# vliu15/3d-brain-tumor-segmentation

Hardware: AMD Instinct MI355X
Metric: training volumes/sec (2ch x 128^3) (higher is better)
Workload: dtype f32; 1 GPU; BASELINE configs[1]: 2ch x 128^3, batch 1 per GPU, fp32, full fwd+bwd with Dice+KL+L2 VAE loss + Dice metric + TF-form Adam; CLI-default model (base_filters=32, depth=4, groups=8, reduction=8; 42,174,773 params); parallelism=dp1, global_batch=1

## Files before the change

### 3d-brain-tumor-segmentation_amd/csrc/conv_wgrad.hip

```cpp
#include <stdlib.h>
#include <type_traits>
#include "common.h"
#include "bts_internal.h"

int bts_prof_on();
void bts_prof_begin(int sym, double flops, hipStream_t stream);
void bts_prof_end(hipStream_t stream);

#define WG_THREADS 512
#define WG_WAVES 8
#define WG_MAXT 4
#define WG_PSLOTS 8
#define WG_QSLOTS 4

struct WgradParams {
  const float* p;
  const float* q;
  float* partial;
  double* partial_b;
  const float* zeros;
  int N, Dp, Hp, Wp, Cp, ldp;
  int Dq, Hq, Wq, Cq, ldq;
  int s, loz, loy, lox;
  int IZ, IY, IX;
// ... 736 lines not shown
      if (c < bestc - 1e-9) { bestc = c; best = n; }
    }
    if (best > p.nsub) best = p.nsub;
    p.sub_per_wg = (int)((p.nsub + best - 1) / best);
    pl.nsp = (p.nsub + p.sub_per_wg - 1) / p.sub_per_wg;
  }
  pl.partial_floats = (long)pl.nsp * pl.npct * pl.nqct * p.ntiles * 1024;
  pl.partial_b_doubles = (long)pl.nsp * pl.nqct * 32;
  return BTS_OK;
}

typedef float wg_f32x2 __attribute__((ext_vector_type(2)));
__device__ __forceinline__ wg_f32x2 wgw_pk_add(wg_f32x2 a, wg_f32x2 b) { wg_f32x2 d; asm("v_pk_add_f32 %0, %1, %2" : "=v"(d) : "v"(a), "v"(b)); return d; }
__device__ __forceinline__ wg_f32x2 wgw_pk_sub(wg_f32x2 a, wg_f32x2 b) { wg_f32x2 d; asm("v_pk_add_f32 %0, %1, %2 neg_lo:[0,1] neg_hi:[0,1]" : "=v"(d) : "v"(a), "v"(b)); return d; }
__device__ __forceinline__ wg_f32x2 wgw_pk_fma(wg_f32x2 a, wg_f32x2 b, wg_f32x2 c) { wg_f32x2 d; asm("v_pk_fma_f32 %0, %1, %2, %3" : "=v"(d) : "v"(a), "v"(b), "v"(c)); return d; }
__device__ __forceinline__ f32x4 wgw_add4(f32x4 a, f32x4 b) { const wg_f32x2 lo = wgw_pk_add(a.xy, b.xy), hi = wgw_pk_add(a.zw, b.zw); return f32x4{lo.x, lo.y, hi.x, hi.y}; }
__device__ __forceinline__ f32x4 wgw_sub4(f32x4 a, f32x4 b) { const wg_f32x2 lo = wgw_pk_sub(a.xy, b.xy), hi = wgw_pk_sub(a.zw, b.zw); return f32x4{lo.x, lo.y, hi.x, hi.y}; }
__device__ __forceinline__ f32x4 wgw_fma4(f32x4 a, wg_f32x2 s, f32x4 c) { const wg_f32x2 lo = wgw_pk_fma(a.xy, s, c.xy), hi = wgw_pk_fma(a.zw, s, c.zw); return f32x4{lo.x, lo.y, hi.x, hi.y}; }
__device__ __forceinline__ float wgw_acc_rd(float a) { float v; asm volatile("v_accvgpr_read_b32 %0, %1" : "=v"(v) : "a"(a)); return v; }

#define WGW_QSTR 28
#define WGW_PTILE (24 * 32 * 16)
#define WGW_QTILE (8 * 32 * WGW_QSTR)
#define WGW_BUF (WGW_PTILE + WGW_QTILE)
#define WGW_NPS 12
#define WGW_NQS 5
#define WGW_THREADS 256

__global__ __launch_bounds__(WGW_THREADS, 1) void wgw_kernel(const WgradParams p) {
  extern __shared__ __attribute__((aligned(16))) float lds[];
  const int tid = threadIdx.x;
  const int lane = tid & 63;
  const int wave = __builtin_amdgcn_readfirstlane(tid >> 6);
  const int ch = lane & 31, hh = lane >> 5;
  const int pct = blockIdx.y, qct = blockIdx.z;
  const float* pP = p.p + pct * 32;
  const float* pQ = p.q + qct * 32;

  const int sxx = tid & 15, scq = (tid >> 4) & 7, srow0 = tid >> 7;
  const int p_lds0 = (srow0 * 32 + scq * 4) * 16 + ((((sxx >> 2) ^ (scq & 3)) << 2) | (sxx & 3));
  unsigned poff[WGW_NPS], pfl0 = 0, pfl1 = 0;
#pragma unroll
  for (int i = 0; i < WGW_NPS; ++i) {
    const int row = srow0 + 2 * i;
    const int zr = row / 6, yr = row - zr * 6;
    poff[i] = (unsigned)(((zr * p.Hp + yr) * p.Wp + sxx) * p.ldp + scq * 4) * 4u;
    const unsigned fl = (zr == 0 ? 1u : 0u) | (zr == 3 ? 2u : 0u) | (yr == 0 ? 4u : 0u) | (yr == 5 ? 8u : 0u);
    if (i < 8) pfl0 |= fl << (4 * i); else pfl1 |= fl << (4 * (i - 8));
  }
  int q_lds[WGW_NQS];
  unsigned qoff[WGW_NQS], qfl = 0;
#pragma unroll
  for (int i = 0; i < WGW_NQS; ++i) {
    const int id = tid + WGW_THREADS * i;
    q_lds[i] = -1; qoff[i] = 0x80000000u;
    if (id < 1152) {
      const int xx = id % 18, kq = (id / 18) & 7, row = id / 144;
      q_lds[i] = WGW_PTILE + (row * 32 + kq * 4) * WGW_QSTR + xx + 3;
      qoff[i] = (unsigned)((((row >> 2) * p.Hq + (row & 3)) * p.Wq + xx) * p.ldq + kq * 4) * 4u;
      qfl |= ((xx == 0 ? 1u : 0u) | (xx == 17 ? 2u : 0u)) << (2 * i);
    }
  }
  int ftx, fty, ftz, fn;
  {
    int t = blockIdx.x * p.sub_per_wg;
    ftx = t % p.ntx; t /= p.ntx;
    fty = t % p.nty; t /= p.nty;
    ftz = t % p.ntz;
    fn = t / p.ntz;
  }
  f32x4 pre[WGW_NPS + WGW_NQS];
  __amdgpu_buffer_rsrc_t f_pr, f_qr;
  unsigned f_tm = 0, f_qm = 0;
  auto fetch_begin = [&]() {
    const int z0 = 2 * ftz, y0 = 4 * fty, x0 = 16 * ftx;
    const float* pb = pP + ((((long)fn * p.Dp + z0 - 1) * p.Hp + y0 - 1) * p.Wp + x0) * p.ldp;
    const float* qb = pQ + ((((long)fn * p.Dq + z0) * p.Hq + y0) * p.Wq + x0 - 1) * p.ldq;
    f_pr = __builtin_amdgcn_make_buffer_rsrc((void*)pb, 0, 0x7fffffff, 0x00020000);
    f_qr = __builtin_amdgcn_make_buffer_rsrc((void*)qb, 0, 0x7fffffff, 0x00020000);
    f_tm = (ftz == 0 ? 1u : 0u) | (ftz == p.ntz - 1 ? 2u : 0u) | (fty == 0 ? 4u : 0u) | (fty == p.nty - 1 ? 8u : 0u);
    f_qm = (ftx == 0 ? 1u : 0u) | (ftx == p.ntx - 1 ? 2u : 0u);
    if (++ftx == p.ntx) { ftx = 0; if (++fty == p.nty) { fty = 0; if (++ftz == p.ntz) { ftz = 0; ++fn; } } }
  };
  auto fetch_p = [&](auto ic) {
    constexpr int i = decltype(ic)::value;
    constexpr int sh = 4 * (i & 7);
    const unsigned fl = (((i < 8 ? pfl0 : pfl1) >> sh) & 15u) & f_tm;
    pre[i] = __builtin_bit_cast(f32x4, __builtin_amdgcn_raw_buffer_load_b128(f_pr, fl ? 0x80000000u : poff[i], 0, 0));
  };
  auto fetch_q = [&](auto ic) {
    constexpr int i = decltype(ic)::value;
    const unsigned fl = ((qfl >> (2 * i)) & 3u) & f_qm;
    pre[WGW_NPS + i] = __builtin_bit_cast(f32x4, __builtin_amdgcn_raw_buffer_load_b128(f_qr, fl ? 0x80000000u : qoff[i], 0, 0));
  };
  auto commit_p = [&](float* buf, auto ic) {
    constexpr int i = decltype(ic)::value;
#pragma unroll
    for (int e = 0; e < 4; ++e) buf[p_lds0 + i * (2 * 32 * 16) + e * 16] = pre[i][e];
  };
  auto commit_q = [&](float* buf, auto ic) {
    constexpr int i = decltype(ic)::value;
    if (q_lds[i] >= 0) {
#pragma unroll
      for (int e = 0; e < 4; ++e) buf[q_lds[i] + e * WGW_QSTR] = pre[WGW_NPS + i][e];
    }
  };
  auto fetch_quarter = [&](auto kc) {
    constexpr int k = decltype(kc)::value;
    fetch_p(IC<3 * k>{}); fetch_p(IC<3 * k + 1>{}); fetch_p(IC<3 * k + 2>{});
    if constexpr (k == 0) { fetch_q(IC<0>{}); fetch_q(IC<1>{}); } else fetch_q(IC<k + 1>{});
  };
  auto commit_quarter = [&](float* buf, auto kc) {
    constexpr int k = decltype(kc)::value;
    commit_p(buf, IC<3 * k>{}); commit_p(buf, IC<3 * k + 1>{}); commit_p(buf, IC<3 * k + 2>{});
    if constexpr (k == 0) { commit_q(buf, IC<0>{}); commit_q(buf, IC<1>{}); } else commit_q(buf, IC<k + 1>{});
  };

  const int ra = (wave == 0) ? 0 : (wave == 2) ? 2 : 1;
  const int rb = (wave == 0) ? 2 : (wave == 1) ? 2 : (wave == 2) ? 1 : 3;
  const float sp = (wave == 1) ? 1.f : -1.f;
  const wg_f32x2 sp2 = {sp, sp};
  const float sq = (wave == 1) ? 1.f : (wave == 2) ? -1.f : 0.f;
  const wg_f32x2 sq2 = {sq, sq};
  const int qX = (wave == 3) ? 4 * 32 * WGW_QSTR : 0;
  const int pswz = (ch >> 2) & 3;
  const int pA = (ra * 6 * 32 + ch) * 16, pB = (rb * 6 * 32 + ch) * 16;
  const bool bias = p.want_bias && pct == 0 && wave == 1;
  double bsum = 0.0;

  f32x16 acc[3][4];
#pragma unroll
  for (int a = 0; a < 3; ++a)
#pragma unroll
    for (int c = 0; c < 4; ++c)
#pragma unroll
      for (int r = 0; r < 16; ++r) acc[a][c][r] = 0.f;

  struct WgwOps {
    f32x4 v[4];
    f32x4 a0, a1, u1, u2;
    float a0s[2], a1s[2], u1s[2], u2s[2];
  };
  auto form = [&](const float* cur, auto stc, WgwOps& o) {
    constexpr int st = decltype(stc)::value;
    constexpr int py2 = st >> 1, sx = st & 1;
    const int xq = 2 * sx + hh;
    const int xo = 4 * xq;
    const int pq = (xq ^ pswz) << 2;
    f32x4 c[4];
#pragma unroll
    for (int yr = 0; yr < 4; ++yr) {
      const f32x4 a = *reinterpret_cast<const f32x4*>(cur + pA + (2 * py2 + yr) * 512 + pq);
      const f32x4 b = *reinterpret_cast<const f32x4*>(cur + pB + (2 * py2 + yr) * 512 + pq);
      c[yr] = wgw_fma4(b, sp2, a);
    }
    o.v[0] = wgw_sub4(c[0], c[2]);
    o.v[1] = wgw_add4(c[1], c[2]);
    o.v[2] = wgw_sub4(c[2], c[1]);
    o.v[3] = wgw_sub4(c[1], c[3]);
    const float* qb = cur + WGW_PTILE + ((2 * py2) * 32 + ch) * WGW_QSTR + xo;
    {
      const f32x4 x0q = *reinterpret_cast<const f32x4*>(qb + qX + 4);
      const f32x4 x1q = *reinterpret_cast<const f32x4*>(qb + qX + 32 * WGW_QSTR + 4);
      const f32x4 y0q = *reinterpret_cast<const f32x4*>(qb + (4 * 32) * WGW_QSTR + 4);
      const f32x4 y1q = *reinterpret_cast<const f32x4*>(qb + (5 * 32) * WGW_QSTR + 4);
      o.a0 = wgw_fma4(y0q, sq2, x0q);
      o.a1 = wgw_fma4(y1q, sq2, x1q);
      o.u1 = wgw_add4(o.a0, o.a1);
      o.u2 = wgw_sub4(o.a0, o.a1);
      if (bias) bsum += (double)((o.u1[0] + o.u1[1]) + (o.u1[2] + o.u1[3]));
    }
#pragma unroll
    for (int e = 0; e < 2; ++e) {
      const int off = e == 0 ? 0 : 8, el = e == 0 ? 3 : 0;
      f32x4 xs0 = *reinterpret_cast<const f32x4*>(qb + qX + off);
      f32x4 xs1 = *reinterpret_cast<const f32x4*>(qb + qX + 32 * WGW_QSTR + off);
      f32x4 ys0 = *reinterpret_cast<const f32x4*>(qb + (4 * 32) * WGW_QSTR + off);
      f32x4 ys1 = *reinterpret_cast<const f32x4*>(qb + (5 * 32) * WGW_QSTR + off);
      asm volatile("" : "+v"(xs0), "+v"(xs1), "+v"(ys0), "+v"(ys1));
      o.a0s[e] = fmaf(ys0[el], sq, xs0[el]);
      o.a1s[e] = fmaf(ys1[el], sq, xs1[el]);
      o.u1s[e] = o.a0s[e] + o.a1s[e];
      o.u2s[e] = o.a0s[e] - o.a1s[e];
    }
  };
  auto mfma48 = [&](const WgwOps& o) {
#pragma unroll
    for (int dx = 0; dx < 3; ++dx)
#pragma unroll
      for (int j = 0; j < 4; ++j) {
        const int w = 5 + j - dx;
        const float b0 = w == 3 ? o.a0s[0] : w == 8 ? o.a0s[1] : o.a0[(w - 4) & 3];
        const float b1 = w == 3 ? o.u1s[0] : w == 8 ? o.u1s[1] : o.u1[(w - 4) & 3];
        const float b2 = w == 3 ? o.u2s[0] : w == 8 ? o.u2s[1] : o.u2[(w - 4) & 3];
        const float b3 = w == 3 ? o.a1s[0] : w == 8 ? o.a1s[1] : o.a1[(w - 4) & 3];
        acc[dx][0] = __builtin_amdgcn_mfma_f32_32x32x2f32(o.v[0][j], b0, acc[dx][0], 0, 0, 0);
        acc[dx][1] = __builtin_amdgcn_mfma_f32_32x32x2f32(o.v[1][j], b1, acc[dx][1], 0, 0, 0);
        acc[dx][2] = __builtin_amdgcn_mfma_f32_32x32x2f32(o.v[2][j], b2, acc[dx][2], 0, 0, 0);
        acc[dx][3] = __builtin_amdgcn_mfma_f32_32x32x2f32(o.v[3][j], b3, acc[dx][3], 0, 0, 0);
      }
  };
#define WGW_SCHED_STEP()                                   \
  _Pragma("unroll") for (int q_ = 0; q_ < 48; ++q_) {      \
    __builtin_amdgcn_sched_group_barrier(0x008, 1, 0);     \
    __builtin_amdgcn_sched_group_barrier(0x002, 2, 0);     \
    __builtin_amdgcn_sched_group_barrier(0x320, 1, 0);     \
  }

  const int t0 = blockIdx.x * p.sub_per_wg;
  int t1 = t0 + p.sub_per_wg;
  if (t1 > p.nsub) t1 = p.nsub;
  if (t0 < t1) {
    fetch_begin();
    fetch_quarter(IC<0>{}); fetch_quarter(IC<1>{}); fetch_quarter(IC<2>{}); fetch_quarter(IC<3>{});
    commit_quarter(lds, IC<0>{}); commit_quarter(lds, IC<1>{}); commit_quarter(lds, IC<2>{}); commit_quarter(lds, IC<3>{});
  }
  __syncthreads();
  WgwOps opA, opB;
  for (int t = t0; t < t1; ++t) {
    const float* cur = lds + ((t - t0) & 1) * WGW_BUF;
    float* nxt = lds + ((t - t0 + 1) & 1) * WGW_BUF;
    const bool more = (t + 1) < t1;
    form(cur, IC<0>{}, opA);
    if (more) fetch_begin();
    __builtin_amdgcn_sched_barrier(0);
    asm volatile("s_nop 3" ::: "memory");
    if (more) fetch_quarter(IC<0>{});
    form(cur, IC<1>{}, opB);
    mfma48(opA);
    WGW_SCHED_STEP();
    __builtin_amdgcn_sched_barrier(0);
    asm volatile("s_nop 1" ::: "memory");
    if (more) { commit_quarter(nxt, IC<0>{}); fetch_quarter(IC<1>{}); }
    form(cur, IC<2>{}, opA);
    mfma48(opB);
    WGW_SCHED_STEP();
    __builtin_amdgcn_sched_barrier(0);
    asm volatile("s_nop 1" ::: "memory");
    if (more) { commit_quarter(nxt, IC<1>{}); fetch_quarter(IC<2>{}); }
    form(cur, IC<3>{}, opB);
    mfma48(opA);
    WGW_SCHED_STEP();
    __builtin_amdgcn_sched_barrier(0);
    asm volatile("s_nop 1" ::: "memory");
    if (more) { commit_quarter(nxt, IC<2>{}); fetch_quarter(IC<3>{}); }
    mfma48(opB);
    WGW_SCHED_STEP();
    __builtin_amdgcn_sched_barrier(0);
    if (more) commit_quarter(nxt, IC<3>{});
    __syncthreads();
  }

  asm volatile("s_nop 15\n\ts_nop 15\n\ts_nop 15\n\ts_nop 15\n\ts_nop 15" ::: "memory");
  float* xl = lds + wave * 9 * 1024;
#pragma unroll
  for (int dx = 0; dx < 3; ++dx)
#pragma unroll
    for (int r = 0; r < 16; ++r) {
      const float u0 = wgw_acc_rd(acc[dx][0][r]), u1 = wgw_acc_rd(acc[dx][1][r]), u2 = wgw_acc_rd(acc[dx][2][r]),
                  u3 = wgw_acc_rd(acc[dx][3][r]);
      const float hs = 0.5f * (u1 + u2), hd = 0.5f * (u1 - u2);
      const int crow = 8 * (r >> 2) + 4 * hh + (r & 3);
      float* o = xl + (dx * 3) * 1024 + crow * 32 + ch;
      o[0] = u0 + hs;
      o[1024] = hd;
      o[2048] = hs - u3;
    }
  __syncthreads();
  float* out = p.partial + ((((long)blockIdx.x * gridDim.y + pct) * gridDim.z + qct) * 27) * 1024;
  for (int e = tid; e < 9 * 1024; e += WGW_THREADS) {
    const int g = e >> 10, ck = e & 1023;
    const int dx = g / 3, ky = g - dx * 3;
    const float l0 = lds[(0 * 9 + g) * 1024 + ck], l1 = lds[(1 * 9 + g) * 1024 + ck], l2 = lds[(2 * 9 + g) * 1024 + ck],
                l3 = lds[(3 * 9 + g) * 1024 + ck];
    const float hs = 0.5f * (l1 + l2), hd = 0.5f * (l1 - l2);
    out[((0 * 3 + ky) * 3 + dx) * 1024 + ck] = l0 + hs;
    out[((1 * 3 + ky) * 3 + dx) * 1024 + ck] = hd;
    out[((2 * 3 + ky) * 3 + dx) * 1024 + ck] = hs - l3;
  }
  if (bias) {
    const double o = __shfl_xor(bsum, 32, 64);
    if (lane < 32) p.partial_b[((long)blockIdx.x * gridDim.z + qct) * 32 + ch] = bsum + o;
  }
}

#define K1W_THREADS 512
#define K1W_U 8
__global__ __launch_bounds__(K1W_THREADS, 2) void k1w_kernel(const WgradParams p, long NV, long chunk) {
  __shared__ float lds[8 * 1024];
  const int tid = threadIdx.x;
  const int lane = tid & 63;
  const int wave = __builtin_amdgcn_readfirstlane(tid >> 6);
  const int ch = lane & 31, hh = lane >> 5;
// ... 63 lines not shown
  r.ntaps = (kind == BTS_CONV_K1) ? 1 : 27;
  r.s = 1; r.neg = 0; r.swapped = 0; r.transposed = 0;
  r.Dp = D; r.Hp = H; r.Wp = W; r.Cp = Cin; r.Dq = D; r.Hq = H; r.Wq = W; r.Cq = Cout;
  if (kind == BTS_CONV_K3S2) {
    if ((D | H | W) & 1) return BTS_ERR_SHAPE;
    r.s = 2; r.Dq = D / 2; r.Hq = H / 2; r.Wq = W / 2;
  } else if (kind == BTS_CONV_K3S2T) {
    r.transposed = 1;
    r.s = 2; r.Dp = 2 * D; r.Hp = 2 * H; r.Wp = 2 * W; r.Cp = Cout; r.Cq = Cin;
  } else if (kind == BTS_CONV_K3S1 && Cout <= 8 && Cin > Cout) {
    r.swapped = 1; r.neg = 1; r.Cp = Cout; r.Cq = Cin;
  }
  return BTS_OK;
}

extern "C" int bts_colsum(const float* x, float* out, void* workspace, long workspace_bytes, int N, long rows, int C,
                          int ld, float scale, int sum_over_n, int accumulate, hipStream_t stream);
extern "C" long bts_colsum_workspace(int N, long rows, int C);

extern "C" long bts_conv3d_bwd_weight_workspace(int kind, int N, int D, int H, int W, int Cin, int Cout) {
  WgradRoles r;
  if (wgrad_roles(r, kind, D, H, W, Cin, Cout) != BTS_OK) return -1;
  WgradPlan pl;
  if (plan_wgrad(pl, r.ntaps, r.s, r.neg, N, r.Dp, r.Hp, r.Wp, r.Cp, r.Dq, r.Hq, r.Wq, r.Cq) != BTS_OK) return -1;
  const long base = ((pl.partial_floats * 4 + pl.partial_b_doubles * 8 + 256 + 15) & ~15L);
  return base + (r.swapped ? bts_colsum_workspace(N, (long)D * H * W, Cout) : 0) + 128;
}

extern "C" int bts_conv3d_bwd_weight(int kind, const float* x, const float* dy, float* dw, float* db, void* workspace,
                                     long workspace_bytes, int N, int D, int H, int W, int Cin, int ldx, int Cout,
                                     int lddy, int dup_start, int dup_shift, int accumulate, hipStream_t stream) {
  WgradRoles ro;
  int r = wgrad_roles(ro, kind, D, H, W, Cin, Cout);
  if (r != BTS_OK) return r;
  if (dup_shift > 0 && (kind == BTS_CONV_K3S2 || kind == BTS_CONV_K3S2T)) return BTS_ERR_UNSUPPORTED;
  WgradPlan pl;
  r = plan_wgrad(pl, ro.ntaps, ro.s, ro.neg, N, ro.Dp, ro.Hp, ro.Wp, ro.Cp, ro.Dq, ro.Hq, ro.Wq, ro.Cq);
  if (r != BTS_OK) return r;
  const long need = bts_conv3d_bwd_weight_workspace(kind, N, D, H, W, Cin, Cout);
  if (workspace_bytes < need || workspace == nullptr) return BTS_ERR_WORKSPACE;
  WgradParams& p = pl.p;
// ... 9 lines not shown
  p.want_bias = (db != nullptr && !pIsDy) ? 1 : 0;
  typedef void (*WgKernel)(const WgradParams);
  static const WgKernel kernels[4] = {wgrad_kernel<0, 0>, wgrad_kernel<1, 0>, wgrad_kernel<2, 1>, wgrad_kernel<2, 2>};
  static bool attr_done = false;
  if (!attr_done) {
    for (int i = 0; i < 4; ++i) {
      hipError_t e = hipFuncSetAttribute(reinterpret_cast<const void*>(kernels[i]), hipFuncAttributeMaxDynamicSharedMemorySize, 160 * 1024);
      if (e != hipSuccess) return (int)e;
    }
    attr_done = true;
  }
  char* ztail = reinterpret_cast<char*>(workspace) + ((need - 64) & ~15L);
  p.zeros = reinterpret_cast<const float*>(ztail);
  const bool glds = (p.ldp % 4 == 0) && (p.Cp % 4 == 0) && ((((uintptr_t)p.p) & 15) == 0) && (p.ldq % 4 == 0) &&
                    (p.Cq % 4 == 0) && ((((uintptr_t)p.q) & 15) == 0);
  if (p.fastf && ((double)p.IZ * p.Hp * p.Wp * p.ldp * 4.0 >= 4.0e9 || (double)p.TZ * p.Hq * p.Wq * p.ldq * 4.0 >= 4.0e9 || !glds))
    p.fastf = p.fixg = 0;
  const bool prof = bts_prof_on();
  if (glds && !p.fastf) {
    hipError_t e = hipMemsetAsync(ztail, 0, 64, stream);
    if (e != hipSuccess) return (int)e;
  }
  const int kidx = !glds ? 0 : (p.fastf ? 1 + p.fixg : 1);
  bool use_wgw = false;
  if (kidx == 2 && ro.ntaps == 27 && ro.s == 1) {
    const char* e = getenv("BTS_WGW");
    use_wgw = !(e && atoi(e) == 0) && 5.0 * p.Hp * p.Wp * p.ldp * 4.0 < 2.0e9 && 3.0 * p.Hq * p.Wq * p.ldq * 4.0 < 2.0e9;
  }
  bool use_k1w = false;
  const long NVall = (long)N * ro.Dq * ro.Hq * ro.Wq;
  if (ro.ntaps == 1 && !pIsDy && p.ntiles == 1 && NVall >= 32768) {
    const char* e = getenv("BTS_K1W");
    use_k1w = !(e && atoi(e) == 0);
  }
  if (use_k1w) {
    const long chunk = (((NVall + pl.nsp - 1) / pl.nsp) + 15) & ~15L;
    if (prof) bts_prof_begin(26, 2.0 * (double)ro.Cp * ro.Cq * (double)NVall, stream);
    (void)hipGetLastError();
    hipLaunchKernelGGL(k1w_kernel, dim3(pl.nsp, pl.npct, pl.nqct), dim3(K1W_THREADS), 0, stream, p, NVall, chunk);
    if (prof) bts_prof_end(stream);
    BTS_LAUNCH_CHECK();
  } else if (use_wgw) {
    static bool wattr = false;
    if (!wattr) {
      hipError_t e = hipFuncSetAttribute(reinterpret_cast<const void*>(wgw_kernel), hipFuncAttributeMaxDynamicSharedMemorySize, 160 * 1024);
      if (e != hipSuccess) return (int)e;
      wattr = true;
    }
    if (prof) bts_prof_begin(24, 2.0 * ro.ntaps * (double)ro.Cp * ro.Cq * (double)N * ro.Dq * ro.Hq * ro.Wq, stream);
    (void)hipGetLastError();
    hipLaunchKernelGGL(wgw_kernel, dim3(pl.nsp, pl.npct, pl.nqct), dim3(WGW_THREADS), (size_t)2 * WGW_BUF * sizeof(float), stream, p);
    if (prof) bts_prof_end(stream);
    BTS_LAUNCH_CHECK();
  } else {
  static const int ksym[4] = {100, 104, 109, 110};
  if (prof) bts_prof_begin(ksym[kidx], 2.0 * ro.ntaps * (double)ro.Cp * ro.Cq * (double)N * ro.Dq * ro.Hq * ro.Wq, stream);
  (void)hipGetLastError(); hipLaunchKernelGGL(kernels[kidx], dim3(pl.nsp, pl.npct, pl.nqct), dim3(WG_THREADS), pl.shmem, stream, p);
// ... 33 lines not shown
```

### 3d-brain-tumor-segmentation_amd/ops.py

```python
import ctypes
import weakref

import numpy as np
import torch

from ._lib import ERRORS, lib

K1, K3S1, K3S2, K3S2T = 0, 1, 2, 3
ROLE_FWD, ROLE_BWD = 0, 1
FLAG_SIGMOID, FLAG_ACCUM = 1, 2
GN_SLAB, GN_CHANNEL = 0, 1

_workspaces = {}

_CFG = {0: '2,1,4,1', 1: '2,2,4,1', 2: '1,2,2,2', 3: '1,1,2,2', 4: '1,1,4,1'}


_VARIANTS = {33: {1: '<0,5>', 2: '<0,4>', 3: '<1,5>', 4: '<1,4>'},
             32: {1: '<3x3x3>', 2: '<1x1x1>'}}


def kernel_symbol(sym, detail=False):
    var, sym = sym >> 16, sym & 0xffff
    if var and detail and sym in _VARIANTS:
# ... 312 lines not shown
        lib().call('bts_conv3d_bwd_data', kind, _p(dy), _p(wp_bwd), _p(dx), _p(ws), nb, n, d, h, w, cin, ld_of(dx), cout,
                   ld_of(dy), FLAG_ACCUM if accumulate else 0, _stream())
    return dx


def conv_bwd_weight(kind, x, dy, dw, db, dup_start=0, dup_shift=0, accumulate=False):
    n, d, h, w, cin = x.shape
    cout = dy.shape[4]
    nb = lib().query('bts_conv3d_bwd_weight_workspace', kind, n, d, h, w, cin, cout)
    ws = workspace(nb, x.device)
    if True:
        lib().call('bts_conv3d_bwd_weight', kind, _p(x), _p(dy), _p(dw), _p(db), _p(ws), nb, n, d, h, w, cin, ld_of(x),
                   cout, ld_of(dy), dup_start, dup_shift, 1 if accumulate else 0, _stream())


def gn_stats(x, groups, mode, eps=1e-5):
    if not x.is_contiguous():
        raise RuntimeError('GroupNormalization statistics need a dense tensor')
    n, c = x.shape[0], x.shape[4]
    v = x.shape[1] * x.shape[2] * x.shape[3]
    nb = lib().query('bts_gn_workspace', n, v, c, groups, mode)
    ws = workspace(nb, x.device)
    mean = torch.empty(n * groups, dtype=torch.float32, device=x.device)
    rstd = torch.empty_like(mean)
    lib().call('bts_gn_stats', _p(x), _p(mean), _p(rstd), _p(ws), nb, n, v, c, groups, mode, eps, _stream())
    return mean, rstd


def gn_apply(x, gamma, beta, mean, rstd, groups, mode, relu, out=None):
    n, c = x.shape[0], x.shape[4]
# ... 1001 lines not shown
```

### include/bts_hip.h

```cpp
#ifndef BTS_HIP_H
#define BTS_HIP_H
#include <stdint.h>
#ifdef __cplusplus
extern "C" {
#endif

typedef struct ihipStream_t* bts_stream_t;

#define BTS_OK 0
#define BTS_ERR_SHAPE (-1)
#define BTS_ERR_ALIGN (-2)
#define BTS_ERR_UNSUPPORTED (-3)
#define BTS_ERR_WORKSPACE (-4)
#define BTS_ERR_RCCL_BASE (-100)

#define BTS_CONV_K1 0
#define BTS_CONV_K3S1 1
#define BTS_CONV_K3S2 2
#define BTS_CONV_K3S2T 3
#define BTS_ROLE_FWD 0
#define BTS_ROLE_BWD_DATA 1
#define BTS_CONV_FLAG_SIGMOID 1
#define BTS_CONV_FLAG_ACCUM 2

// ... 17 lines not shown
int bts_conv3d_fwd_can_fuse(int N, int D, int H, int W, int Cin, int Cout);
int bts_conv3d_fwd_fused2(const float* x, const float* wp_fwd, const float* bias, float* y, const float* wp2,
                          const float* bias2, float* y2, int N, int D, int H, int W, int Cin, int ldx, int Cout, int ldy,
                          int ldy2, bts_stream_t stream);
long bts_conv3d_bwd_data_workspace(int kind, int N, int D, int H, int W, int Cin, int Cout);
int bts_conv3d_bwd_data(int kind, const float* dy, const float* wp_bwd, float* dx, void* workspace, long workspace_bytes,
                        int N, int D, int H, int W, int Cin, int lddx, int Cout, int lddy, int flags, bts_stream_t stream);
int bts_conv3d_fwd_config(int kind, int N, int D, int H, int W, int Cin, int Cout);
int bts_conv3d_bwd_data_config(int kind, int N, int D, int H, int W, int Cin, int Cout);
int bts_conv3d_kernel(int dir, int kind, int N, int D, int H, int W, int Cin, int ldx, int Cout, int ldy, int flags, int second,
                      int ld2, int G, int aligned, long workspace_bytes);
long bts_conv3d_bwd_weight_workspace(int kind, int N, int D, int H, int W, int Cin, int Cout);
int bts_conv3d_bwd_weight(int kind, const float* x, const float* dy, float* dw, float* db, void* workspace,
                          long workspace_bytes, int N, int D, int H, int W, int Cin, int ldx, int Cout, int lddy,
                          int dup_start, int dup_shift, int accumulate, bts_stream_t stream);

long bts_gn_workspace(int N, long V, int C, int G, int mode);
long bts_gn_bwd_workspace(int N, long V, int C, int G, int mode);
int bts_gn_stats(const float* x, float* mean, float* rstd, void* workspace, long workspace_bytes, int N, long V, int C,
                 int G, int mode, float eps, bts_stream_t stream);
int bts_gn_apply(const float* x, float* y, const float* gamma, const float* beta, const float* mean, const float* rstd,
                 int N, long V, int C, int ldy, int G, int mode, int relu, bts_stream_t stream);
int bts_gn_bwd(const float* x, const float* dy, float* dx, const float* gamma, const float* beta, const float* mean,
               const float* rstd, float* dgamma, float* dbeta, void* workspace, long workspace_bytes, int N, long V, int C,
               int lddy, int G, int mode, int relu, int accumulate_params, bts_stream_t stream);

long bts_colsum_workspace(int N, long rows, int C);
int bts_colsum(const float* x, float* out, void* workspace, long workspace_bytes, int N, long rows, int C, int ld,
               float scale, int sum_over_n, int accumulate, bts_stream_t stream);
int bts_se_mlp_fwd(const float* gap, const float* w1, const float* w2, float* h, float* ch, int N, int F, int R,
// ... 292 lines not shown
```

Baseline: 27.12 volumes/s.

## Use 2D Winograd F(2,3) in y and x for the wgrad MFMA kernel

Reworks the Winograd weight-gradient kernel so the transform covers both y and x, replacing the old y-only transform plus three direct x taps. Each stage now issues 16 MFMAs instead of 48, and the output transform is applied twice in the epilogue. The LDS tile layout changes to an unswizzled 18-wide row stride, and the p tile now carries the x halo instead of q. The prefetch pipeline is restructured so loads run unconditionally against a zero-size buffer descriptor when no tile remains. It also adds a form-probe API exposed to Python. The main risks are extra transform ALU work, possible LDS bank conflicts from the new layout, and numerical differences.

```diff
diff --git a/3d-brain-tumor-segmentation_amd/csrc/conv_wgrad.hip b/3d-brain-tumor-segmentation_amd/csrc/conv_wgrad.hip
--- a/3d-brain-tumor-segmentation_amd/csrc/conv_wgrad.hip
+++ b/3d-brain-tumor-segmentation_amd/csrc/conv_wgrad.hip
@@ -774,18 +774,16 @@
 __device__ __forceinline__ wg_f32x2 wgw_pk_add(wg_f32x2 a, wg_f32x2 b) { wg_f32x2 d; asm("v_pk_add_f32 %0, %1, %2" : "=v"(d) : "v"(a), "v"(b)); return d; }
 __device__ __forceinline__ wg_f32x2 wgw_pk_sub(wg_f32x2 a, wg_f32x2 b) { wg_f32x2 d; asm("v_pk_add_f32 %0, %1, %2 neg_lo:[0,1] neg_hi:[0,1]" : "=v"(d) : "v"(a), "v"(b)); return d; }
 __device__ __forceinline__ wg_f32x2 wgw_pk_fma(wg_f32x2 a, wg_f32x2 b, wg_f32x2 c) { wg_f32x2 d; asm("v_pk_fma_f32 %0, %1, %2, %3" : "=v"(d) : "v"(a), "v"(b), "v"(c)); return d; }
-__device__ __forceinline__ f32x4 wgw_add4(f32x4 a, f32x4 b) { const wg_f32x2 lo = wgw_pk_add(a.xy, b.xy), hi = wgw_pk_add(a.zw, b.zw); return f32x4{lo.x, lo.y, hi.x, hi.y}; }
-__device__ __forceinline__ f32x4 wgw_sub4(f32x4 a, f32x4 b) { const wg_f32x2 lo = wgw_pk_sub(a.xy, b.xy), hi = wgw_pk_sub(a.zw, b.zw); return f32x4{lo.x, lo.y, hi.x, hi.y}; }
-__device__ __forceinline__ f32x4 wgw_fma4(f32x4 a, wg_f32x2 s, f32x4 c) { const wg_f32x2 lo = wgw_pk_fma(a.xy, s, c.xy), hi = wgw_pk_fma(a.zw, s, c.zw); return f32x4{lo.x, lo.y, hi.x, hi.y}; }
+__device__ __forceinline__ wg_f32x2 wgw_pk_addsub(wg_f32x2 a, wg_f32x2 b) { wg_f32x2 d; asm("v_pk_add_f32 %0, %1, %2 op_sel:[0,1] op_sel_hi:[0,1] neg_hi:[0,1]" : "=v"(d) : "v"(a), "v"(b)); return d; }
 __device__ __forceinline__ float wgw_acc_rd(float a) { float v; asm volatile("v_accvgpr_read_b32 %0, %1" : "=v"(v) : "a"(a)); return v; }
 
-#define WGW_QSTR 28
-#define WGW_PTILE (24 * 32 * 16)
-#define WGW_QTILE (8 * 32 * WGW_QSTR)
+#define WGW_THREADS 256
+#define WGW_RS 18
+#define WGW_PTILE (24 * 32 * WGW_RS)
+#define WGW_QTILE (8 * 32 * WGW_RS)
 #define WGW_BUF (WGW_PTILE + WGW_QTILE)
-#define WGW_NPS 12
-#define WGW_NQS 5
-#define WGW_THREADS 256
+#define WGW_NPS 14
+#define WGW_NQS 4
 
 __global__ __launch_bounds__(WGW_THREADS, 1) void wgw_kernel(const WgradParams p) {
   extern __shared__ __attribute__((aligned(16))) float lds[];
@@ -797,33 +795,40 @@
   const float* pP = p.p + pct * 32;
   const float* pQ = p.q + qct * 32;
 
-  const int sxx = tid & 15, scq = (tid >> 4) & 7, srow0 = tid >> 7;
-  const int p_lds0 = (srow0 * 32 + scq * 4) * 16 + ((((sxx >> 2) ^ (scq & 3)) << 2) | (sxx & 3));
-  unsigned poff[WGW_NPS], pfl0 = 0, pfl1 = 0;
+  int p_lds[WGW_NPS];
+  unsigned poff[WGW_NPS], pfl[3] = {0u, 0u, 0u};
 #pragma unroll
   for (int i = 0; i < WGW_NPS; ++i) {
-    const int row = srow0 + 2 * i;
-    const int zr = row / 6, yr = row - zr * 6;
-    poff[i] = (unsigned)(((zr * p.Hp + yr) * p.Wp + sxx) * p.ldp + scq * 4) * 4u;
-    const unsigned fl = (zr == 0 ? 1u : 0u) | (zr == 3 ? 2u : 0u) | (yr == 0 ? 4u : 0u) | (yr == 5 ? 8u : 0u);
-    if (i < 8) pfl0 |= fl << (4 * i); else pfl1 |= fl << (4 * (i - 8));
+    const int id = tid + WGW_THREADS * i;
+    const int idle = id - 24 * 18 * 8;
+    p_lds[i] = WGW_PTILE + ((idle >> 4) * 32 + ((idle >> 1) & 7) * 4) * WGW_RS + 16 + (idle & 1);
+    poff[i] = 0x80000000u;
+    if (id < 24 * 18 * 8) {
+      const int cq = id & 7, vox = id >> 3;
+      const int row = vox / 18, xx = vox - row * 18;
+      const int zr = row / 6, yr = row - zr * 6;
+      p_lds[i] = (row * 32 + cq * 4) * WGW_RS + xx;
+      poff[i] = (unsigned)(((zr * p.Hp + yr) * p.Wp + xx) * p.ldp + cq * 4) * 4u;
+      const unsigned fl = (zr == 0 ? 1u : 0u) | (zr == 3 ? 2u : 0u) | (yr == 0 ? 4u : 0u) | (yr == 5 ? 8u : 0u) |
+                          (xx == 0 ? 16u : 0u) | (xx == 17 ? 32u : 0u);
+      pfl[i / 5] |= fl << (6 * (i % 5));
+    }
   }
   int q_lds[WGW_NQS];
-  unsigned qoff[WGW_NQS], qfl = 0;
+  unsigned qoff[WGW_NQS];
 #pragma unroll
   for (int i = 0; i < WGW_NQS; ++i) {
     const int id = tid + WGW_THREADS * i;
-    q_lds[i] = -1; qoff[i] = 0x80000000u;
-    if (id < 1152) {
-      const int xx = id % 18, kq = (id / 18) & 7, row = id / 144;
-      q_lds[i] = WGW_PTILE + (row * 32 + kq * 4) * WGW_QSTR + xx + 3;
-      qoff[i] = (unsigned)((((row >> 2) * p.Hq + (row & 3)) * p.Wq + xx) * p.ldq + kq * 4) * 4u;
-      qfl |= ((xx == 0 ? 1u : 0u) | (xx == 17 ? 2u : 0u)) << (2 * i);
-    }
-  }
+    const int cq = id & 7, xx = (id >> 3) & 15, row = id >> 7;
+    q_lds[i] = WGW_PTILE + (row * 32 + cq * 4) * WGW_RS + xx;
+    qoff[i] = (unsigned)((((row >> 2) * p.Hq + (row & 3)) * p.Wq + xx) * p.ldq + cq * 4) * 4u;
+  }
+  const int t0 = blockIdx.x * p.sub_per_wg;
+  int t1 = t0 + p.sub_per_wg;
+  if (t1 > p.nsub) t1 = p.nsub;
   int ftx, fty, ftz, fn;
   {
-    int t = blockIdx.x * p.sub_per_wg;
+    int t = t0;
     ftx = t % p.ntx; t /= p.ntx;
     fty = t % p.nty; t /= p.nty;
     ftz = t % p.ntz;
@@ -831,49 +836,49 @@
   }
   f32x4 pre[WGW_NPS + WGW_NQS];
   __amdgpu_buffer_rsrc_t f_pr, f_qr;
-  unsigned f_tm = 0, f_qm = 0;
-  auto fetch_begin = [&]() {
+  unsigned f_tm = 0;
+  auto fetch_begin = [&](bool live) {
     const int z0 = 2 * ftz, y0 = 4 * fty, x0 = 16 * ftx;
-    const float* pb = pP + ((((long)fn * p.Dp + z0 - 1) * p.Hp + y0 - 1) * p.Wp + x0) * p.ldp;
-    const float* qb = pQ + ((((long)fn * p.Dq + z0) * p.Hq + y0) * p.Wq + x0 - 1) * p.ldq;
-    f_pr = __builtin_amdgcn_make_buffer_rsrc((void*)pb, 0, 0x7fffffff, 0x00020000);
-    f_qr = __builtin_amdgcn_make_buffer_rsrc((void*)qb, 0, 0x7fffffff, 0x00020000);
-    f_tm = (ftz == 0 ? 1u : 0u) | (ftz == p.ntz - 1 ? 2u : 0u) | (fty == 0 ? 4u : 0u) | (fty == p.nty - 1 ? 8u : 0u);
-    f_qm = (ftx == 0 ? 1u : 0u) | (ftx == p.ntx - 1 ? 2u : 0u);
-    if (++ftx == p.ntx) { ftx = 0; if (++fty == p.nty) { fty = 0; if (++ftz == p.ntz) { ftz = 0; ++fn; } } }
-  };
-  auto fetch_p = [&](auto ic) {
+    const float* pb = pP + ((((long)fn * p.Dp + z0 - 1) * p.Hp + y0 - 1) * p.Wp + x0 - 1) * p.ldp;
+    const float* qb = pQ + ((((long)fn * p.Dq + z0) * p.Hq + y0) * p.Wq + x0) * p.ldq;
+    f_pr = __builtin_amdgcn_make_buffer_rsrc((void*)pb, 0, live ? 0x7fffffff : 0, 0x00020000);
+    f_qr = __builtin_amdgcn_make_buffer_rsrc((void*)qb, 0, live ? 0x7fffffff : 0, 0x00020000);
+    f_tm = (ftz == 0 ? 1u : 0u) | (ftz == p.ntz - 1 ? 2u : 0u) | (fty == 0 ? 4u : 0u) | (fty == p.nty - 1 ? 8u : 0u) |
+           (ftx == 0 ? 16u : 0u) | (ftx == p.ntx - 1 ? 32u : 0u);
+    const int cx = (ftx + 1 == p.ntx) ? 1 : 0;
+    ftx = cx ? 0 : ftx + 1;
+    const int cy = (fty + cx == p.nty) ? 1 : 0;
+    fty = cy ? 0 : fty + cx;
+    const int cz = (ftz + cy == p.ntz) ? 1 : 0;
+    ftz = cz ? 0 : ftz + cy;
+    fn += cz;
+  };
+  auto fetch_slot = [&](auto ic) {
     constexpr int i = decltype(ic)::value;
-    constexpr int sh = 4 * (i & 7);
-    const unsigned fl = (((i < 8 ? pfl0 : pfl1) >> sh) & 15u) & f_tm;
-    pre[i] = __builtin_bit_cast(f32x4, __builtin_amdgcn_raw_buffer_load_b128(f_pr, fl ? 0x80000000u : poff[i], 0, 0));
-  };
-  auto fetch_q = [&](auto ic) {
+    if constexpr (i < WGW_NPS) {
+      const unsigned fl = ((pfl[i / 5] >> (6 * (i % 5))) & 63u) & f_tm;
+      pre[i] = __builtin_bit_cast(f32x4, __builtin_amdgcn_raw_buffer_load_b128(f_pr, fl ? 0x80000000u : poff[i], 0, 0));
+    } else {
+      pre[i] = __builtin_bit_cast(f32x4, __builtin_amdgcn_raw_buffer_load_b128(f_qr, qoff[i - WGW_NPS], 0, 0));
+    }
+  };
+  auto commit_slot = [&](float* buf, auto ic) {
     constexpr int i = decltype(ic)::value;
-    const unsigned fl = ((qfl >> (2 * i)) & 3u) & f_qm;
-    pre[WGW_NPS + i] = __builtin_bit_cast(f32x4, __builtin_amdgcn_raw_buffer_load_b128(f_qr, fl ? 0x80000000u : qoff[i], 0, 0));
-  };
-  auto commit_p = [&](float* buf, auto ic) {
-    constexpr int i = decltype(ic)::value;
-#pragma unroll
-    for (int e = 0; e < 4; ++e) buf[p_lds0 + i * (2 * 32 * 16) + e * 16] = pre[i][e];
-  };
-  auto commit_q = [&](float* buf, auto ic) {
-    constexpr int i = decltype(ic)::value;
-    if (q_lds[i] >= 0) {
-#pragma unroll
-      for (int e = 0; e < 4; ++e) buf[q_lds[i] + e * WGW_QSTR] = pre[WGW_NPS + i][e];
-    }
-  };
-  auto fetch_quarter = [&](auto kc) {
+    if constexpr (i < WGW_NPS) {
+#pragma unroll
+      for (int e = 0; e < 4; ++e) buf[p_lds[i] + e * WGW_RS] = pre[i][e];
+    } else {
+#pragma unroll
+      for (int e = 0; e < 4; ++e) buf[q_lds[i - WGW_NPS] + e * WGW_RS] = pre[i][e];
+    }
+  };
+  auto fetch_group = [&](auto kc) {
     constexpr int k = decltype(kc)::value;
-    fetch_p(IC<3 * k>{}); fetch_p(IC<3 * k + 1>{}); fetch_p(IC<3 * k + 2>{});
-    if constexpr (k == 0) { fetch_q(IC<0>{}); fetch_q(IC<1>{}); } else fetch_q(IC<k + 1>{});
-  };
-  auto commit_quarter = [&](float* buf, auto kc) {
+    fetch_slot(IC<3 * k>{}); fetch_slot(IC<3 * k + 1>{}); fetch_slot(IC<3 * k + 2>{});
+  };
+  auto commit_group = [&](float* buf, auto kc) {
     constexpr int k = decltype(kc)::value;
-    commit_p(buf, IC<3 * k>{}); commit_p(buf, IC<3 * k + 1>{}); commit_p(buf, IC<3 * k + 2>{});
-    if constexpr (k == 0) { commit_q(buf, IC<0>{}); commit_q(buf, IC<1>{}); } else commit_q(buf, IC<k + 1>{});
+    commit_slot(buf, IC<3 * k>{}); commit_slot(buf, IC<3 * k + 1>{}); commit_slot(buf, IC<3 * k + 2>{});
   };
 
   const int ra = (wave == 0) ? 0 : (wave == 2) ? 2 : 1;
@@ -882,161 +887,158 @@
   const wg_f32x2 sp2 = {sp, sp};
   const float sq = (wave == 1) ? 1.f : (wave == 2) ? -1.f : 0.f;
   const wg_f32x2 sq2 = {sq, sq};
-  const int qX = (wave == 3) ? 4 * 32 * WGW_QSTR : 0;
-  const int pswz = (ch >> 2) & 3;
-  const int pA = (ra * 6 * 32 + ch) * 16, pB = (rb * 6 * 32 + ch) * 16;
+  const int pA = (ra * 6 * 32 + ch) * WGW_RS + 2 * hh, pB = (rb * 6 * 32 + ch) * WGW_RS + 2 * hh;
+  const int qXa = WGW_PTILE + ((wave == 3 ? 4 : 0) * 32 + ch) * WGW_RS + 2 * hh;
+  const int qYa = WGW_PTILE + (4 * 32 + ch) * WGW_RS + 2 * hh;
   const bool bias = p.want_bias && pct == 0 && wave == 1;
   double bsum = 0.0;
-
-  f32x16 acc[3][4];
-#pragma unroll
-  for (int a = 0; a < 3; ++a)
+  float bs = 0.f;
+
+  f32x16 acc[4][4];
+#pragma unroll
+  for (int a = 0; a < 4; ++a)
 #pragma unroll
     for (int c = 0; c < 4; ++c)
 #pragma unroll
       for (int r = 0; r < 16; ++r) acc[a][c][r] = 0.f;
 
-  struct WgwOps {
-    f32x4 v[4];
-    f32x4 a0, a1, u1, u2;
-    float a0s[2], a1s[2], u1s[2], u2s[2];
-  };
+  struct WgwOps { float v[4][4], t[4][4]; };
   auto form = [&](const float* cur, auto stc, WgwOps& o) {
     constexpr int st = decltype(stc)::value;
-    constexpr int py2 = st >> 1, sx = st & 1;
-    const int xq = 2 * sx + hh;
-    const int xo = 4 * xq;
-    const int pq = (xq ^ pswz) << 2;
-    f32x4 c[4];
+    constexpr int py = st >> 2, sx = st & 3;
+    wg_f32x2 cl[4], cx[4];
 #pragma unroll
     for (int yr = 0; yr < 4; ++yr) {
-      const f32x4 a = *reinterpret_cast<const f32x4*>(cur + pA + (2 * py2 + yr) * 512 + pq);
-      const f32x4 b = *reinterpret_cast<const f32x4*>(cur + pB + (2 * py2 + yr) * 512 + pq);
-      c[yr] = wgw_fma4(b, sp2, a);
-    }
-    o.v[0] = wgw_sub4(c[0], c[2]);
-    o.v[1] = wgw_add4(c[1], c[2]);
-    o.v[2] = wgw_sub4(c[2], c[1]);
-    o.v[3] = wgw_sub4(c[1], c[3]);
-    const float* qb = cur + WGW_PTILE + ((2 * py2) * 32 + ch) * WGW_QSTR + xo;
-    {
-      const f32x4 x0q = *reinterpret_cast<const f32x4*>(qb + qX + 4);
-      const f32x4 x1q = *reinterpret_cast<const f32x4*>(qb + qX + 32 * WGW_QSTR + 4);
-      const f32x4 y0q = *reinterpret_cast<const f32x4*>(qb + (4 * 32) * WGW_QSTR + 4);
-      const f32x4 y1q = *reinterpret_cast<const f32x4*>(qb + (5 * 32) * WGW_QSTR + 4);
-      o.a0 = wgw_fma4(y0q, sq2, x0q);
-      o.a1 = wgw_fma4(y1q, sq2, x1q);
-      o.u1 = wgw_add4(o.a0, o.a1);
-      o.u2 = wgw_sub4(o.a0, o.a1);
-      if (bias) bsum += (double)((o.u1[0] + o.u1[1]) + (o.u1[2] + o.u1[3]));
-    }
-#pragma unroll
-    for (int e = 0; e < 2; ++e) {
-      const int off = e == 0 ? 0 : 8, el = e == 0 ? 3 : 0;
-      f32x4 xs0 = *reinterpret_cast<const f32x4*>(qb + qX + off);
-      f32x4 xs1 = *reinterpret_cast<const f32x4*>(qb + qX + 32 * WGW_QSTR + off);
-      f32x4 ys0 = *reinterpret_cast<const f32x4*>(qb + (4 * 32) * WGW_QSTR + off);
-      f32x4 ys1 = *reinterpret_cast<const f32x4*>(qb + (5 * 32) * WGW_QSTR + off);
-      asm volatile("" : "+v"(xs0), "+v"(xs1), "+v"(ys0), "+v"(ys1));
-      o.a0s[e] = fmaf(ys0[el], sq, xs0[el]);
-      o.a1s[e] = fmaf(ys1[el], sq, xs1[el]);
-      o.u1s[e] = o.a0s[e] + o.a1s[e];
-      o.u2s[e] = o.a0s[e] - o.a1s[e];
-    }
-  };
-  auto mfma48 = [&](const WgwOps& o) {
-#pragma unroll
-    for (int dx = 0; dx < 3; ++dx)
-#pragma unroll
-      for (int j = 0; j < 4; ++j) {
-        const int w = 5 + j - dx;
-        const float b0 = w == 3 ? o.a0s[0] : w == 8 ? o.a0s[1] : o.a0[(w - 4) & 3];
-        const float b1 = w == 3 ? o.u1s[0] : w == 8 ? o.u1s[1] : o.u1[(w - 4) & 3];
-        const float b2 = w == 3 ? o.u2s[0] : w == 8 ? o.u2s[1] : o.u2[(w - 4) & 3];
-        const float b3 = w == 3 ? o.a1s[0] : w == 8 ? o.a1s[1] : o.a1[(w - 4) & 3];
-        acc[dx][0] = __builtin_amdgcn_mfma_f32_32x32x2f32(o.v[0][j], b0, acc[dx][0], 0, 0, 0);
-        acc[dx][1] = __builtin_amdgcn_mfma_f32_32x32x2f32(o.v[1][j], b1, acc[dx][1], 0, 0, 0);
-        acc[dx][2] = __builtin_amdgcn_mfma_f32_32x32x2f32(o.v[2][j], b2, acc[dx][2], 0, 0, 0);
-        acc[dx][3] = __builtin_amdgcn_mfma_f32_32x32x2f32(o.v[3][j], b3, acc[dx][3], 0, 0, 0);
-      }
+      const float* a = cur + pA + (2 * py + yr) * 32 * WGW_RS + 4 * sx;
+      const float* b = cur + pB + (2 * py + yr) * 32 * WGW_RS + 4 * sx;
+      cl[yr] = wgw_pk_fma(*reinterpret_cast<const wg_f32x2*>(b), sp2, *reinterpret_cast<const wg_f32x2*>(a));
+      cx[yr] = wgw_pk_fma(*reinterpret_cast<const wg_f32x2*>(b + 2), sp2, *reinterpret_cast<const wg_f32x2*>(a + 2));
+    }
+    wg_f32x2 vl[4], vx[4];
+    vl[0] = wgw_pk_sub(cl[0], cl[2]); vx[0] = wgw_pk_sub(cx[0], cx[2]);
+    vl[1] = wgw_pk_add(cl[1], cl[2]); vx[1] = wgw_pk_add(cx[1], cx[2]);
+    vl[2] = wgw_pk_sub(cl[2], cl[1]); vx[2] = wgw_pk_sub(cx[2], cx[1]);
+    vl[3] = wgw_pk_sub(cl[1], cl[3]); vx[3] = wgw_pk_sub(cx[1], cx[3]);
+#pragma unroll
+    for (int a = 0; a < 4; ++a) {
+      const wg_f32x2 d = wgw_pk_sub(vl[a], vx[a]), m = wgw_pk_addsub(vx[a], vl[a]);
+      o.v[a][0] = d.x;
+      o.v[a][1] = m.x;
+      o.v[a][2] = m.y;
+      o.v[a][3] = d.y;
+    }
+    wg_f32x2 qa[2];
+#pragma unroll
+    for (int yr = 0; yr < 2; ++yr) {
+      const wg_f32x2 X = *reinterpret_cast<const wg_f32x2*>(cur + qXa + (2 * py + yr) * 32 * WGW_RS + 4 * sx);
+      const wg_f32x2 Y = *reinterpret_cast<const wg_f32x2*>(cur + qYa + (2 * py + yr) * 32 * WGW_RS + 4 * sx);
+      qa[yr] = wgw_pk_fma(Y, sq2, X);
+    }
+    const wg_f32x2 ty[4] = {qa[0], wgw_pk_add(qa[0], qa[1]), wgw_pk_sub(qa[0], qa[1]), qa[1]};
+#pragma unroll
+    for (int a = 0; a < 4; ++a) {
+      const wg_f32x2 m = wgw_pk_addsub(ty[a], ty[a]);
+      o.t[a][0] = ty[a].x;
+      o.t[a][1] = m.x;
+      o.t[a][2] = m.y;
+      o.t[a][3] = ty[a].y;
+    }
+    bs += o.t[1][1];
+  };
+  auto mfma16 = [&](const WgwOps& o) {
+#pragma unroll
+    for (int a = 0; a < 4; ++a)
+#pragma unroll
+      for (int b = 0; b < 4; ++b) acc[a][b] = __builtin_amdgcn_mfma_f32_32x32x2f32(o.v[a][b], o.t[a][b], acc[a][b], 0, 0, 0);
   };
 #define WGW_SCHED_STEP()                                   \
-  _Pragma("unroll") for (int q_ = 0; q_ < 48; ++q_) {      \
+  _Pragma("unroll") for (int q_ = 0; q_ < 16; ++q_) {      \
     __builtin_amdgcn_sched_group_barrier(0x008, 1, 0);     \
-    __builtin_amdgcn_sched_group_barrier(0x002, 2, 0);     \
-    __builtin_amdgcn_sched_group_barrier(0x320, 1, 0);     \
-  }
-
-  const int t0 = blockIdx.x * p.sub_per_wg;
-  int t1 = t0 + p.sub_per_wg;
-  if (t1 > p.nsub) t1 = p.nsub;
-  if (t0 < t1) {
-    fetch_begin();
-    fetch_quarter(IC<0>{}); fetch_quarter(IC<1>{}); fetch_quarter(IC<2>{}); fetch_quarter(IC<3>{});
-    commit_quarter(lds, IC<0>{}); commit_quarter(lds, IC<1>{}); commit_quarter(lds, IC<2>{}); commit_quarter(lds, IC<3>{});
-  }
+    __builtin_amdgcn_sched_group_barrier(0x002, 4, 0);     \
+    __builtin_amdgcn_sched_group_barrier(0x320, 3, 0);     \
+  }
+#define WGW_STEP_END()                       \
+  WGW_SCHED_STEP();                          \
+  __builtin_amdgcn_sched_barrier(0);         \
+  asm volatile("s_nop 1" ::: "memory");
+
+  fetch_begin(t0 < t1);
+  fetch_group(IC<0>{}); fetch_group(IC<1>{}); fetch_group(IC<2>{}); fetch_group(IC<3>{}); fetch_group(IC<4>{}); fetch_group(IC<5>{});
+  commit_group(lds, IC<0>{}); commit_group(lds, IC<1>{}); commit_group(lds, IC<2>{}); commit_group(lds, IC<3>{});
+  commit_group(lds, IC<4>{}); commit_group(lds, IC<5>{});
   __syncthreads();
   WgwOps opA, opB;
+  form(lds, IC<0>{}, opA);
+  fetch_begin((t0 + 1) < t1);
+  __builtin_amdgcn_sched_barrier(0);
+  asm volatile("s_nop 3" ::: "memory");
   for (int t = t0; t < t1; ++t) {
     const float* cur = lds + ((t - t0) & 1) * WGW_BUF;
     float* nxt = lds + ((t - t0 + 1) & 1) * WGW_BUF;
-    const bool more = (t + 1) < t1;
-    form(cur, IC<0>{}, opA);
-    if (more) fetch_begin();
+    form(cur, IC<1>{}, opB); fetch_group(IC<0>{});
+    mfma16(opA);
+    WGW_STEP_END();
+    form(cur, IC<2>{}, opA); commit_group(nxt, IC<0>{}); fetch_group(IC<1>{});
+    mfma16(opB);
+    WGW_STEP_END();
+    form(cur, IC<3>{}, opB); commit_group(nxt, IC<1>{}); fetch_group(IC<2>{});
+    mfma16(opA);
+    WGW_STEP_END();
+    form(cur, IC<4>{}, opA); commit_group(nxt, IC<2>{}); fetch_group(IC<3>{});
+    mfma16(opB);
+    WGW_STEP_END();
+    form(cur, IC<5>{}, opB); commit_group(nxt, IC<3>{}); fetch_group(IC<4>{});
+    mfma16(opA);
+    WGW_STEP_END();
+    form(cur, IC<6>{}, opA); commit_group(nxt, IC<4>{}); fetch_group(IC<5>{});
+    mfma16(opB);
+    WGW_STEP_END();
+    form(cur, IC<7>{}, opB); commit_group(nxt, IC<5>{});
+    mfma16(opA);
+    WGW_STEP_END();
+    bsum += (double)bs;
+    bs = 0.f;
+    __syncthreads();
     __builtin_amdgcn_sched_barrier(0);
-    asm volatile("s_nop 3" ::: "memory");
-    if (more) fetch_quarter(IC<0>{});
-    form(cur, IC<1>{}, opB);
-    mfma48(opA);
-    WGW_SCHED_STEP();
-    __builtin_amdgcn_sched_barrier(0);
-    asm volatile("s_nop 1" ::: "memory");
-    if (more) { commit_quarter(nxt, IC<0>{}); fetch_quarter(IC<1>{}); }
-    form(cur, IC<2>{}, opA);
-    mfma48(opB);
-    WGW_SCHED_STEP();
-    __builtin_amdgcn_sched_barrier(0);
-    asm volatile("s_nop 1" ::: "memory");
-    if (more) { commit_quarter(nxt, IC<1>{}); fetch_quarter(IC<2>{}); }
-    form(cur, IC<3>{}, opB);
-    mfma48(opA);
-    WGW_SCHED_STEP();
-    __builtin_amdgcn_sched_barrier(0);
-    asm volatile("s_nop 1" ::: "memory");
-    if (more) { commit_quarter(nxt, IC<2>{}); fetch_quarter(IC<3>{}); }
-    mfma48(opB);
-    WGW_SCHED_STEP();
-    __builtin_amdgcn_sched_barrier(0);
-    if (more) commit_quarter(nxt, IC<3>{});
-    __syncthreads();
+    form(nxt, IC<0>{}, opA);
+    fetch_begin((t + 2) < t1);
+    mfma16(opB);
+    WGW_STEP_END();
   }
 
   asm volatile("s_nop 15\n\ts_nop 15\n\ts_nop 15\n\ts_nop 15\n\ts_nop 15" ::: "memory");
+  __syncthreads();
   float* xl = lds + wave * 9 * 1024;
 #pragma unroll
-  for (int dx = 0; dx < 3; ++dx)
-#pragma unroll
-    for (int r = 0; r < 16; ++r) {
-      const float u0 = wgw_acc_rd(acc[dx][0][r]), u1 = wgw_acc_rd(acc[dx][1][r]), u2 = wgw_acc_rd(acc[dx][2][r]),
-                  u3 = wgw_acc_rd(acc[dx][3][r]);
+  for (int r = 0; r < 16; ++r) {
+    float m[3][4];
+#pragma unroll
+    for (int b = 0; b < 4; ++b) {
+      const float u0 = wgw_acc_rd(acc[0][b][r]), u1 = wgw_acc_rd(acc[1][b][r]), u2 = wgw_acc_rd(acc[2][b][r]),
+                  u3 = wgw_acc_rd(acc[3][b][r]);
       const float hs = 0.5f * (u1 + u2), hd = 0.5f * (u1 - u2);
-      const int crow = 8 * (r >> 2) + 4 * hh + (r & 3);
-      float* o = xl + (dx * 3) * 1024 + crow * 32 + ch;
-      o[0] = u0 + hs;
-      o[1024] = hd;
-      o[2048] = hs - u3;
-    }
+      m[0][b] = u0 + hs;
+      m[1][b] = hd;
+      m[2][b] = hs - u3;
+    }
+    const int crow = 8 * (r >> 2) + 4 * hh + (r & 3);
+    float* o = xl + crow * 32 + ch;
+#pragma unroll
+    for (int ky = 0; ky < 3; ++ky) {
+      const float hs = 0.5f * (m[ky][1] + m[ky][2]), hd = 0.5f * (m[ky][1] - m[ky][2]);
+      o[(ky * 3 + 0) * 1024] = m[ky][0] + hs;
+      o[(ky * 3 + 1) * 1024] = hd;
+      o[(ky * 3 + 2) * 1024] = hs - m[ky][3];
+    }
+  }
   __syncthreads();
   float* out = p.partial + ((((long)blockIdx.x * gridDim.y + pct) * gridDim.z + qct) * 27) * 1024;
   for (int e = tid; e < 9 * 1024; e += WGW_THREADS) {
-    const int g = e >> 10, ck = e & 1023;
-    const int dx = g / 3, ky = g - dx * 3;
-    const float l0 = lds[(0 * 9 + g) * 1024 + ck], l1 = lds[(1 * 9 + g) * 1024 + ck], l2 = lds[(2 * 9 + g) * 1024 + ck],
-                l3 = lds[(3 * 9 + g) * 1024 + ck];
+    const float l0 = lds[0 * 9 * 1024 + e], l1 = lds[1 * 9 * 1024 + e], l2 = lds[2 * 9 * 1024 + e], l3 = lds[3 * 9 * 1024 + e];
     const float hs = 0.5f * (l1 + l2), hd = 0.5f * (l1 - l2);
-    out[((0 * 3 + ky) * 3 + dx) * 1024 + ck] = l0 + hs;
-    out[((1 * 3 + ky) * 3 + dx) * 1024 + ck] = hd;
-    out[((2 * 3 + ky) * 3 + dx) * 1024 + ck] = hs - l3;
+    out[0 * 9 * 1024 + e] = l0 + hs;
+    out[1 * 9 * 1024 + e] = hd;
+    out[2 * 9 * 1024 + e] = hs - l3;
   }
   if (bias) {
     const double o = __shfl_xor(bsum, 32, 64);
@@ -1130,6 +1132,20 @@
   return BTS_OK;
 }
 
+static int wgrad_variant(WgradParams& p, bool vec) {
+  if (p.fastf && ((double)p.IZ * p.Hp * p.Wp * p.ldp * 4.0 >= 4.0e9 || (double)p.TZ * p.Hq * p.Wq * p.ldq * 4.0 >= 4.0e9 || !vec))
+    p.fastf = p.fixg = 0;
+  return !vec ? 0 : (p.fastf ? 1 + p.fixg : 1);
+}
+enum { BTS_FORM_DIRECT = 0, BTS_FORM_WG2 = 2, BTS_FORM_WG3 = 3 };
+static int wgrad_form(const WgradParams& p, const WgradRoles& ro, int variant) {
+  if (variant != 2 || ro.ntaps != 27 || ro.s != 1) return BTS_FORM_DIRECT;
+  const char* e = getenv("BTS_WGW");
+  if (e && atoi(e) == 0) return BTS_FORM_DIRECT;
+  if (!(5.0 * p.Hp * p.Wp * p.ldp * 4.0 < 2.0e9 && 3.0 * p.Hq * p.Wq * p.ldq * 4.0 < 2.0e9)) return BTS_FORM_DIRECT;
+  return BTS_FORM_WG3;
+}
+
 extern "C" int bts_colsum(const float* x, float* out, void* workspace, long workspace_bytes, int N, long rows, int C,
                           int ld, float scale, int sum_over_n, int accumulate, hipStream_t stream);
 extern "C" long bts_colsum_workspace(int N, long rows, int C);
@@ -1141,6 +1157,21 @@
   if (plan_wgrad(pl, r.ntaps, r.s, r.neg, N, r.Dp, r.Hp, r.Wp, r.Cp, r.Dq, r.Hq, r.Wq, r.Cq) != BTS_OK) return -1;
   const long base = ((pl.partial_floats * 4 + pl.partial_b_doubles * 8 + 256 + 15) & ~15L);
   return base + (r.swapped ? bts_colsum_workspace(N, (long)D * H * W, Cout) : 0) + 128;
+}
+
+extern "C" int bts_conv3d_bwd_weight_form(int kind, int N, int D, int H, int W, int Cin, int ldx, int Cout, int lddy, int aligned) {
+  WgradRoles ro;
+  int r = wgrad_roles(ro, kind, D, H, W, Cin, Cout);
+  if (r != BTS_OK) return r;
+  WgradPlan pl;
+  r = plan_wgrad(pl, ro.ntaps, ro.s, ro.neg, N, ro.Dp, ro.Hp, ro.Wp, ro.Cp, ro.Dq, ro.Hq, ro.Wq, ro.Cq);
+  if (r != BTS_OK) return r;
+  WgradParams& p = pl.p;
+  const bool pIsDy = ro.transposed || ro.swapped;
+  p.ldp = pIsDy ? lddy : ldx;
+  p.ldq = pIsDy ? ldx : lddy;
+  const bool vec = (p.ldp % 4 == 0) && (p.Cp % 4 == 0) && (p.ldq % 4 == 0) && (p.Cq % 4 == 0) && (aligned & 3) == 3;
+  return wgrad_form(p, ro, wgrad_variant(p, vec));
 }
 
 extern "C" int bts_conv3d_bwd_weight(int kind, const float* x, const float* dy, float* dw, float* db, void* workspace,
@@ -1180,18 +1211,12 @@
   p.zeros = reinterpret_cast<const float*>(ztail);
   const bool glds = (p.ldp % 4 == 0) && (p.Cp % 4 == 0) && ((((uintptr_t)p.p) & 15) == 0) && (p.ldq % 4 == 0) &&
                     (p.Cq % 4 == 0) && ((((uintptr_t)p.q) & 15) == 0);
-  if (p.fastf && ((double)p.IZ * p.Hp * p.Wp * p.ldp * 4.0 >= 4.0e9 || (double)p.TZ * p.Hq * p.Wq * p.ldq * 4.0 >= 4.0e9 || !glds))
-    p.fastf = p.fixg = 0;
+  const int kidx = wgrad_variant(p, glds);
+  const int form = wgrad_form(p, ro, kidx);
   const bool prof = bts_prof_on();
   if (glds && !p.fastf) {
     hipError_t e = hipMemsetAsync(ztail, 0, 64, stream);
     if (e != hipSuccess) return (int)e;
-  }
-  const int kidx = !glds ? 0 : (p.fastf ? 1 + p.fixg : 1);
-  bool use_wgw = false;
-  if (kidx == 2 && ro.ntaps == 27 && ro.s == 1) {
-    const char* e = getenv("BTS_WGW");
-    use_wgw = !(e && atoi(e) == 0) && 5.0 * p.Hp * p.Wp * p.ldp * 4.0 < 2.0e9 && 3.0 * p.Hq * p.Wq * p.ldq * 4.0 < 2.0e9;
   }
   bool use_k1w = false;
   const long NVall = (long)N * ro.Dq * ro.Hq * ro.Wq;
@@ -1206,7 +1231,7 @@
     hipLaunchKernelGGL(k1w_kernel, dim3(pl.nsp, pl.npct, pl.nqct), dim3(K1W_THREADS), 0, stream, p, NVall, chunk);
     if (prof) bts_prof_end(stream);
     BTS_LAUNCH_CHECK();
-  } else if (use_wgw) {
+  } else if (form != BTS_FORM_DIRECT) {
     static bool wattr = false;
     if (!wattr) {
       hipError_t e = hipFuncSetAttribute(reinterpret_cast<const void*>(wgw_kernel), hipFuncAttributeMaxDynamicSharedMemorySize, 160 * 1024);
diff --git a/3d-brain-tumor-segmentation_amd/ops.py b/3d-brain-tumor-segmentation_amd/ops.py
--- a/3d-brain-tumor-segmentation_amd/ops.py
+++ b/3d-brain-tumor-segmentation_amd/ops.py
@@ -350,6 +350,12 @@
                    cout, ld_of(dy), dup_start, dup_shift, 1 if accumulate else 0, _stream())
 
 
+def conv_bwd_weight_form(kind, x, dy):
+    n, d, h, w, cin = x.shape
+    aligned = (1 if x.data_ptr() % 16 == 0 else 0) | (2 if dy.data_ptr() % 16 == 0 else 0)
+    return lib().probe('bts_conv3d_bwd_weight_form', kind, n, d, h, w, cin, ld_of(x), dy.shape[4], ld_of(dy), aligned)
+
+
 def gn_stats(x, groups, mode, eps=1e-5):
     if not x.is_contiguous():
         raise RuntimeError('GroupNormalization statistics need a dense tensor')
diff --git a/include/bts_hip.h b/include/bts_hip.h
--- a/include/bts_hip.h
+++ b/include/bts_hip.h
@@ -55,6 +55,7 @@
 int bts_conv3d_bwd_weight(int kind, const float* x, const float* dy, float* dw, float* db, void* workspace,
                           long workspace_bytes, int N, int D, int H, int W, int Cin, int ldx, int Cout, int lddy,
                           int dup_start, int dup_shift, int accumulate, bts_stream_t stream);
+int bts_conv3d_bwd_weight_form(int kind, int N, int D, int H, int W, int Cin, int ldx, int Cout, int lddy, int aligned);
 
 long bts_gn_workspace(int N, long V, int C, int G, int mode);
 long bts_gn_bwd_workspace(int N, long V, int C, int G, int mode);
```

Measured after the change: 28.13 volumes/s, median of 6. 3.8% higher.
